# 20242204033/RIS-VEC-MARL

Hardware: AMD Instinct MI355X
Metric: env-steps/sec (all agents) at 8 veh x 64 RIS (higher is better)
Workload: dtype f32

## Files before the change

### ris_vec_marl_amd/csrc/k_step_gen.hip

```cpp
#include <cstddef>

#include "risvec_pipe.hpp"

#ifndef RISVEC_GEN_STORES
#define RISVEC_GEN_STORES kStNonTemporal
#endif

#ifndef RISVEC_GEN_EARLY
#define RISVEC_GEN_EARLY 1
#endif

#ifndef RISVEC_GEN_PRIO
#define RISVEC_GEN_PRIO 1
#endif

#ifndef RISVEC_GEN_STAMPS
#define RISVEC_GEN_STAMPS 0
#endif

namespace risvec {

using GenStores = StorePolicy<RISVEC_GEN_STORES>;
constexpr bool kGenEarlyDraw = RISVEC_GEN_EARLY != 0;
constexpr int kGenPrio = RISVEC_GEN_PRIO;
constexpr bool kGenStamps = RISVEC_GEN_STAMPS != 0;
static_assert(kGenPrio >= 0 && kGenPrio <= 3, "RISVEC_GEN_PRIO: 0 (none) or schedule 1, 2, 3");

constexpr int gen_prio_level(int schedule, int NL, int done) {
    if (schedule == 3) return done < (NL + 1) / 2 ? 1 : 0;
    if (schedule == 2 && done == NL) return 3;
    const int top = NL < 3 ? NL : 3;
    return schedule == 0 || done >= top ? 0 : top - done;
}

constexpr int gen_prio_change(int schedule, int NL, int done) {
    if (schedule == 0) return -1;
    const int now = gen_prio_level(schedule, NL, done);
    return done == 0 || now != gen_prio_level(schedule, NL, done - 1) ? now : -1;
}

template <int V, int M, class Core>
constexpr int gen_prio_of() {
    return std::is_same<Core, MarlCore>::value && V == 8 && M == 64 ? kGenPrio : 0;
}

constexpr int gen_leaf_rank(int G, int NP, int J) {
    auto rev = [](int G_, int j) {
        int r = 0;
        for (int b = 1; b < G_ / 8; b <<= 1) r = (r << 1) | ((j & b) ? 1 : 0);
        return r;
    };
    int rank = 0;
    for (int j = 0; j < G / 8; ++j)
        if (8 * j < NP && rev(G, j) < rev(G, J)) ++rank;
    return rank;
}
constexpr int gen_leaf_count(int G, int NP) { return (NP < G ? NP : G) / 8; }

#if RISVEC_GEN_STAMPS
constexpr int kGenStampSlots = 16, kGenStampMax = 12;
__device__ unsigned long long* g_gen_stamps = nullptr;
__device__ long long g_gen_stamps_waves = 0;
struct GenStamps {
    unsigned long long t[kGenStampMax];
    unsigned long long rt0;
    int n = 0;
    __device__ __forceinline__ void mark() { t[n++] = __builtin_amdgcn_s_memtime(); }
};
#else
struct GenStamps {
    __device__ __forceinline__ void mark() {}
};
#endif

template <int V, int M>
struct GenShape : PipeShape<V, M> {
    using S = PipeShape<V, M>;
    static_assert(M % kGeoChunk == 0, "rows are rebuilt in whole 16-element chunks");
    static_assert(S::EPW * V == kWave, "a group is 64 rows");
    static constexpr int NCH = M / kGeoChunk;
    static_assert(NCH <= kWave, "a pass must cover at least one row");
    static constexpr int RPP = kWave / NCH;
    static constexpr int RPU = S::PC * S::VPP;
    static_assert(RPP % RPU == 0, "a pass must hold whole units");
    static constexpr int UPP = RPP / RPU;
    static constexpr int SP = UPP >= S::CHUNKS ? 1 : S::CHUNKS / UPP;
    static constexpr int EPO = SP * UPP / S::CHUNKS;
    static constexpr int NO = NCH / SP;
    static_assert(SP * UPP % S::CHUNKS == 0 && NCH % SP == 0 && NO * EPO == S::EPW, "outer iterations must tile the group");
    static constexpr int STAGE = kWave * (kGeoChunk / 2 + 1);
};

template <int SP, bool HD>
struct GenRows {
    double ang[SP];
    double2 w[SP];
};
template <int SP>
struct GenRows<SP, true> {
    double2 head[SP];
    double2 w[SP];
};
template <int SP, int EPO, int NIT, bool TK, bool HD>
struct GenFeed : GenRows<SP, HD> {
    float4 t[EPO][NIT];
};
template <int SP, int EPO, int NIT, bool HD>
struct GenFeed<SP, EPO, NIT, true, HD> : GenRows<SP, HD> {
    unsigned k[EPO][NIT];
};

template <class Core>
struct GenArgs {
    Dims d;
    typename Core::Params P;
    typename Core::Args A;
    const double* steer;
    const double* z_r;
    int n_groups_total, per_wave, rev;
};

template <class Core>
__device__ __forceinline__ const GenArgs<Core>& late_args() {
    static_assert(offsetof(GenArgs<Core>, d) == 0 && std::is_trivially_copyable<GenArgs<Core>>::value,
                  "the kernel-argument segment must be the struct itself");
    typedef const __attribute__((address_space(4))) GenArgs<Core>* SegPtr;
    SegPtr seg = (SegPtr)__builtin_amdgcn_kernarg_segment_ptr();
    asm volatile("" : "+s"(seg));
    return *(const GenArgs<Core>*)seg;
}

template <int V, int M, class Core, bool TK, bool ONE, bool HD>
__device__ __forceinline__ void gen_stage_form(const GenArgs<Core>& KA) {
    using In = typename Core::In;
    using S = GenShape<V, M>;
    constexpr int VP = S::VP, EPW = S::EPW, NP = S::NP, G = S::G, NIT = S::NIT, VPP = S::VPP;
    constexpr int PC = S::PC, CHUNKS = S::CHUNKS, K = S::K;
    constexpr int NCH = S::NCH, RPP = S::RPP, RPU = S::RPU, UPP = S::UPP, SP = S::SP, EPO = S::EPO, NO = S::NO;
    static_assert(std::is_same<typename Core::Args, StepArgs>::value, "the GEN members step on StepArgs");
    using Feed = GenFeed<SP, EPO, NIT, TK, HD>;
    __shared__ float s_img[kBlock / kWave][kWave * 2];
    __shared__ float2 s_ph[TK ? kBlock / kWave : 1][16];
    __shared__ float4 s_stage[kBlock / kWave][S::STAGE];

    const Dims& d = KA.d;
    const typename Core::Args& A = KA.A;
    const double* __restrict__ steer = KA.steer;
    const int n_groups_total = KA.n_groups_total;

    const int lane = threadIdx.x & (kWave - 1), wave = threadIdx.x >> 6;
    const int gl = lane % G, gv = lane / G;
    const int wid = __builtin_amdgcn_readfirstlane(blockIdx.x * (kBlock / kWave) + wave);
    const float4* __restrict__ t4 = reinterpret_cast<const float4*>(A.theta);
    const float4* __restrict__ b4 = reinterpret_cast<const float4*>(A.b);
    const double2* __restrict__ z2 = reinterpret_cast<const double2*>(KA.z_r);
    const int e_last = d.E - 1;
    const int row_last = d.E * V - 1;
    float4 bq[NIT];
    int pcl[NIT];
#pragma unroll
    for (int it = 0; it < NIT; ++it) {
        const int p = gl + it * G;
        const float4 x = b4[p < NP ? p : NP - 1];
        bq[it] = p < NP ? x : make_float4(0.f, 0.f, 0.f, 0.f);
        pcl[it] = (NP % G == 0 || p < NP) ? p : NP - 1;
    }
    const int p_row = lane / NCH, p_ch = lane % NCH, p_m0 = p_ch * kGeoChunk;
    float4* __restrict__ stage = s_stage[wave];
    float4* __restrict__ p_dst = stage + lane * (kGeoChunk / 2 + 1);
    const float4* c_src[NIT];
#pragma unroll
    for (int it = 0; it < NIT; ++it) {
        const int f = gv * NP + pcl[it];
        c_src[it] = stage + (f >> 3) * (kGeoChunk / 2 + 1) + (f & 7);
    }

    auto load_feed = [&](Feed& f, int grp, int o) {
#pragma unroll
        for (int sp = 0; sp < SP; ++sp) {
            int row = grp * kWave + (o * SP + sp) * RPP + p_row;
            row = row < row_last ? row : row_last;
            if constexpr (HD) f.head[sp] = reinterpret_cast<const double2*>(steer)[(long long)row * NCH + p_ch];
            else f.ang[sp] = steer[row];
            f.w[sp] = z2[row];
        }
#pragma unroll
        for (int ie = 0; ie < EPO; ++ie) {
            int e = grp * EPW + o * EPO + ie;
            e = e < e_last ? e : e_last;
            if constexpr (TK) {
                const uint8_t* __restrict__ kb = A.theta_k + (long long)e * A.theta_k_stride;
#pragma unroll
                for (int it = 0; it < NIT; ++it) f.k[ie][it] = *reinterpret_cast<const uint16_t*>(kb + 2 * pcl[it]);
            } else {
                const float4* __restrict__ tb = t4 + (long long)e * NP;
#pragma unroll
                for (int it = 0; it < NIT; ++it) f.t[ie][it] = tb[pcl[it]];
            }
        }
    };

    auto do_outer = [&](int o, const Feed& cur) {
        float2 w0[NIT], w1[NIT];
#pragma unroll
        for (int sp = 0; sp < SP; ++sp) {
            float4 q[kGeoChunk / 2];
            if constexpr (HD) steer_chunk_from_head(cur.head[sp].x, cur.head[sp].y, cur.w[sp].x, cur.w[sp].y, q);
            else steer_chunk(cur.ang[sp], cur.w[sp].x, cur.w[sp].y, p_m0, q);
#pragma unroll
            for (int k = 0; k < kGeoChunk / 2; ++k) p_dst[k] = q[k];
            __builtin_amdgcn_wave_barrier();
#pragma unroll
            for (int ul = 0; ul < UPP; ++ul) {
                const int uo = sp * UPP + ul;
                const int c = uo % CHUNKS, ie = uo / CHUNKS;
                if (c == 0) {
#pragma unroll
                    for (int it = 0; it < NIT; ++it) {
                        float2 t0, t1;
                        if constexpr (TK) {
                            t0 = s_ph[wave][cur.k[ie][it] & 15u];
                            t1 = s_ph[wave][(cur.k[ie][it] >> 8) & 15u];
                        } else {
                            t0 = make_float2(cur.t[ie][it].x, cur.t[ie][it].y);
                            t1 = make_float2(cur.t[ie][it].z, cur.t[ie][it].w);
                        }
                        w0[it] = cmul(t0, make_float2(bq[it].x, bq[it].y));
                        w1[it] = cmul(t1, make_float2(bq[it].z, bq[it].w));
                    }
                }
                float val[8];
#pragma unroll
                for (int pc = 0; pc < PC; ++pc) {
                    float2 acc = make_float2(0.f, 0.f);
#pragma unroll
                    for (int it = 0; it < NIT; ++it) {
                        const float4 h = c_src[it][((ul * RPU + pc * VPP) * NCH) * (kGeoChunk / 2 + 1)];
                        acc = cfma(make_float2(h.x, h.y), w0[it], acc);
                        acc = cfma(make_float2(h.z, h.w), w1[it], acc);
                    }
                    val[2 * pc] = acc.x;
                    val[2 * pc + 1] = acc.y;
                }
                treduce<K, G / 2>(val, gl);
                if (gl % S::WSTRIDE == 0) {
                    const int j = gl / S::WSTRIDE;
                    const int v = (c * PC + (j >> 1)) * VPP + gv;
                    const int i = o * EPO + ie;
                    s_img[wave][(i * VP + v) * 2 + (j & 1)] = val[0];
                }
            }
            __builtin_amdgcn_wave_barrier();
        }
    };

    const int v_mine = lane % VP;

    if constexpr (ONE) {
        if constexpr (TK) {
            RISVEC_ARGS_IN_ONE_TRIP("s"(steer), "s"(KA.z_r), "s"(A.theta_k), "s"(A.theta_k_stride), "s"(A.b),
                                    "s"(n_groups_total), "s"(d.E));
        } else {
            RISVEC_ARGS_IN_ONE_TRIP("s"(steer), "s"(KA.z_r), "s"(A.theta), "s"(A.b), "s"(n_groups_total), "s"(d.E));
        }
        const int grp = wid;
        if (grp >= n_groups_total) return;
        Feed cur;
        load_feed(cur, grp, 0);
        if constexpr (TK) {
            theta_table_fill(s_ph[wave], lane);
            __builtin_amdgcn_wave_barrier();
        }
        const int e_mine = grp * EPW + lane / VP;
        const bool active = e_mine < d.E;
        const In in = Core::load(d, A, e_mine, v_mine, active);
        Core::hold(in);
#pragma unroll 1
        for (int o = 0; o + 1 < NO; ++o) {
            Feed nx;
            load_feed(nx, grp, o + 1);
            do_outer(o, cur);
            cur = nx;
        }
        do_outer(NO - 1, cur);

        const GenArgs<Core>& L = late_args<Core>();
        __builtin_amdgcn_wave_barrier();
        const float2 img = *reinterpret_cast<const float2*>(&s_img[wave][lane * 2]);
        Core::template run<VP, GenStores>(L.d, L.P, L.A, e_mine, v_mine, active, img, in);
    } else {
        const int per_wave = KA.per_wave;
        const int nw = gridDim.x * (kBlock / kWave);
        const int stride = per_wave > 0 ? 1 : nw;
        int grp = per_wave > 0 ? wid * per_wave : wid;
        int grp_end = per_wave > 0 ? grp + per_wave : n_groups_total;
        grp_end = grp_end < n_groups_total ? grp_end : n_groups_total;
        if constexpr (TK) {
            RISVEC_ARGS_IN_ONE_TRIP("s"(steer), "s"(KA.z_r), "s"(A.theta_k), "s"(A.theta_k_stride), "s"(A.b),
                                    "s"(n_groups_total), "s"(per_wave), "s"(d.E));
        } else {
            RISVEC_ARGS_IN_ONE_TRIP("s"(steer), "s"(KA.z_r), "s"(A.theta), "s"(A.b), "s"(n_groups_total), "s"(per_wave),
                                    "s"(d.E));
        }
        if (grp >= grp_end) return;
        const int grp_first = grp;
        if (KA.rev) {
            while (grp + stride < grp_end) grp += stride;
        }
        const int step = KA.rev ? -stride : stride;
        Feed cur;
        load_feed(cur, grp, 0);
        if constexpr (TK) {
            theta_table_fill(s_ph[wave], lane);
            __builtin_amdgcn_wave_barrier();
        }

        auto do_group = [&](int g_cur, const In& in, In& in_nx) {
            const int g_nx = g_cur + step;
            const int nxt = (g_nx >= grp_first && g_nx < grp_end) ? g_nx : 0;
            const int e_mine = g_cur * EPW + lane / VP;
            const bool active = e_mine < d.E;
            Core::hold(in);

#pragma unroll 1
            for (int o = 0; o < NO; ++o) {
                Feed nx;
                if (o + 1 < NO) load_feed(nx, g_cur, o + 1);
                else load_feed(nx, nxt, 0);
                do_outer(o, cur);
                cur = nx;
            }
            const GenArgs<Core>& L = late_args<Core>();
            in_nx = Core::load(L.d, L.A, nxt * EPW + lane / VP, v_mine, nxt * EPW + lane / VP < L.d.E);

            __builtin_amdgcn_wave_barrier();
            const float2 img = *reinterpret_cast<const float2*>(&s_img[wave][lane * 2]);
            Core::template run<VP, GenStores>(L.d, L.P, L.A, e_mine, v_mine, active, img, in);
            __builtin_amdgcn_wave_barrier();
        };

        In inA = Core::load(d, A, grp * EPW + lane / VP, v_mine, grp * EPW + lane / VP < d.E), inB;
        while (true) {
            do_group(grp, inA, inB);
            grp += step;
            if (grp < grp_first || grp >= grp_end) break;
            do_group(grp, inB, inA);
            grp += step;
            if (grp < grp_first || grp >= grp_end) break;
        }
    }
}

template <int G, int O, int J, class Leaf>
__device__ __forceinline__ void row_tree_block(float2 (&out)[8], Leaf&& leaf) {
    if constexpr (O == G) {
        leaf(std::integral_constant<int, J>{}, out);
    } else if constexpr (O >= 16) {
        float2 far[8];
        row_tree_block<G, 2 * O, J>(out, leaf);
        row_tree_block<G, 2 * O, J + O / 8>(far, leaf);
#pragma unroll
        for (int k = 0; k < 8; ++k) out[k] = make_float2(out[k].x + far[k].x, out[k].y + far[k].y);
    } else {
        static_assert(O == 8 && J == 0, "below 16 the values of a row sit in one block");
        float2 far[8];
        row_tree_block<G, 16, 0>(out, leaf);
        row_tree_block<G, 16, 1>(far, leaf);
#pragma unroll
        for (int k = 0; k < 8; ++k) out[k] = make_float2(out[k].x + far[7 - k].x, out[k].y + far[7 - k].y);
    }
}

template <int G, class Leaf>
__device__ __forceinline__ float2 row_tree(Leaf&& leaf) {
    static_assert(G == 16 || G == 32 || G == 64, "treduce<K, G/2> starts at distance 8, 16 or 32");
    float2 s[8];
    row_tree_block<G, 8, 0>(s, leaf);
#pragma unroll
    for (int g = 0; g < 4; ++g) s[g] = make_float2(s[g].x + s[7 - g].x, s[g].y + s[7 - g].y);
#pragma unroll
    for (int g = 0; g < 2; ++g) s[g] = make_float2(s[g].x + s[g + 2].x, s[g].y + s[g + 2].y);
    return make_float2(s[0].x + s[1].x, s[0].y + s[1].y);
}

template <int Q>
struct alignas(2 * Q) GenIdx {
    unsigned w[Q / 2];
};

template <int V, int M, class Core, bool TK, bool HD>
__device__ __forceinline__ void gen_row_lane_form(const GenArgs<Core>& KA) {
    using In = typename Core::In;
    using S = GenShape<V, M>;
    constexpr int VP = S::VP, EPW = S::EPW, NP = S::NP, G = S::G, NIT = S::NIT, NCH = S::NCH;
    static_assert(std::is_same<typename Core::Args, StepArgs>::value, "the GEN members step on StepArgs");
    static_assert(VP == V && EPW * V == kWave, "lane = row of the group");
    static_assert(NP % V == 0 && (NP / V) % 2 == 0, "an env's w is made by its V lanes, an even share each");
    static_assert(NP % G == 0 || NIT == 1, "ragged rows: whole blocks past the end of the row");
    constexpr int Q = NP / V;
    constexpr int WS = NP + 1;
    __shared__ float4 s_w[kBlock / kWave][EPW * WS];
    __shared__ float2 s_ph[TK ? kBlock / kWave : 1][16];

    const Dims& d = KA.d;
    const typename Core::Args& A = KA.A;
    const double* __restrict__ steer = KA.steer;
    const int n_groups_total = KA.n_groups_total;

    constexpr int NL = gen_leaf_count(G, NP);
    constexpr int PRIO = gen_prio_of<V, M, Core>();
    [[maybe_unused]] GenStamps ts;
    if constexpr (kGenStamps) {
#if RISVEC_GEN_STAMPS
        ts.rt0 = __builtin_amdgcn_s_memrealtime();
#endif
        ts.mark();
    }

    const int lane = threadIdx.x & (kWave - 1), wave = threadIdx.x >> 6;
    const int wid = __builtin_amdgcn_readfirstlane(blockIdx.x * (kBlock / kWave) + wave);
    constexpr int level0 = gen_prio_change(PRIO, NL, 0);
#define RISVEC_GEN_ENTRY(text, ...)                                                                                        \
    if constexpr (TK) {                                                                                                    \
        asm volatile(text ::"s"(steer), "s"(KA.z_r), "s"(A.theta_k), "s"(A.theta_k_stride), "s"(A.b), "s"(n_groups_total), \
                     "s"(d.E)__VA_ARGS__);                                                                                 \
    } else {                                                                                                               \
        asm volatile(text ::"s"(steer), "s"(KA.z_r), "s"(A.theta), "s"(A.b), "s"(n_groups_total), "s"(d.E)__VA_ARGS__);    \
    }
    if constexpr (level0 >= 0) {
        RISVEC_GEN_ENTRY("s_setprio %[level]", , [level] "n"(level0))
    } else {
        RISVEC_GEN_ENTRY("", )
    }
#undef RISVEC_GEN_ENTRY
    const int grp = wid;
    if (grp >= n_groups_total) return;

    const int v_mine = lane % VP, i_env = lane / VP;
    const int e_mine = grp * EPW + i_env;
    const bool active = e_mine < d.E;
    const int e_ld = active ? e_mine : d.E - 1;
    const int row = e_ld * V + v_mine;
    double2 head[HD ? NCH : 1];
    if constexpr (HD) {
#pragma unroll
        for (int c = 0; c < NCH; ++c) head[c] = reinterpret_cast<const double2*>(steer)[(long long)row * NCH + c];
    } else {
        head[0].x = steer[row];
    }
    const double2 z = reinterpret_cast<const double2*>(KA.z_r)[row];
    GenIdx<Q> kq;
    float4 tq[TK ? 1 : Q], bq[Q];
    if constexpr (TK) {
        kq = *reinterpret_cast<const GenIdx<Q>*>(A.theta_k + (long long)e_ld * A.theta_k_stride + 2 * Q * v_mine);
    } else {
        const float4* __restrict__ tb = reinterpret_cast<const float4*>(A.theta) + (long long)e_ld * NP + Q * v_mine;
#pragma unroll
        for (int i = 0; i < Q; ++i) tq[i] = tb[i];
    }
#pragma unroll
    for (int i = 0; i < Q; ++i) bq[i] = reinterpret_cast<const float4*>(A.b)[Q * v_mine + i];
    if constexpr (TK) {
        theta_table_fill(s_ph[wave], lane);
        __builtin_amdgcn_wave_barrier();
    }
    RISVEC_ARGS_IN_ONE_TRIP("s"(A.action), "s"(A.data_buf), "s"(A.partner), "s"(A.arrivals), "s"(A.n_groups), "s"(A.mec_q),
                            "s"(A.pl), "s"(A.flags), "s"(d.V), "s"(d.env_offset), "s"(A.seed), "s"(A.counter),
                            "s"(KA.P.poisson_cdf[0]), "s"(KA.P.poisson_cdf[1]), "s"(KA.P.poisson_cdf[2]),
                            "s"(KA.P.poisson_cdf[3]), "s"(KA.P.poisson_cdf[4]), "s"(KA.P.poisson_cdf[5]),
                            "s"(KA.P.poisson_cdf[6]), "s"(KA.P.poisson_cdf[7]));
    const In in = Core::load(d, A, e_mine, v_mine, active);
    int arr = 0;
    if constexpr (kGenEarlyDraw) {
        arr = Core::draw(d, KA.P, A, e_mine, v_mine);
        asm volatile("" : "+v"(arr));
    }
    Core::hold(in);
    if constexpr (kGenStamps) {
        if constexpr (TK) asm volatile("" : "+v"(kq.w[0]), "+v"(bq[0].x));
        else asm volatile("" : "+v"(tq[0].x), "+v"(bq[0].x));
        ts.mark();
    }

    float4* __restrict__ wrow = s_w[wave] + i_env * WS;
#pragma unroll
    for (int i = 0; i < Q; ++i) {
        float2 t0, t1;
        if constexpr (TK) {
            const unsigned k2 = kq.w[i / 2] >> (16 * (i & 1));
            t0 = s_ph[wave][k2 & 15u];
            t1 = s_ph[wave][(k2 >> 8) & 15u];
        } else {
            t0 = make_float2(tq[i].x, tq[i].y);
            t1 = make_float2(tq[i].z, tq[i].w);
        }
        const float2 w0 = cmul(t0, make_float2(bq[i].x, bq[i].y));
        const float2 w1 = cmul(t1, make_float2(bq[i].z, bq[i].w));
        wrow[Q * v_mine + i] = make_float4(w0.x, w0.y, w1.x, w1.y);
    }
    __builtin_amdgcn_wave_barrier();

    auto leaf = [&](auto jc, float2 (&acc)[8]) {
        constexpr int J = decltype(jc)::value;
#pragma unroll
        for (int k = 0; k < 8; ++k) acc[k] = make_float2(0.f, 0.f);
        if constexpr (8 * J < NP) {
#pragma unroll
            for (int it = 0; it < NIT; ++it) {
                constexpr int GC = G / 8;
                const int c = J + it * GC;
                float4 q[kGeoChunk / 2];
                if constexpr (HD) steer_chunk_from_head(head[c].x, head[c].y, z.x, z.y, q);
                else steer_chunk(head[0].x, z.x, z.y, c * kGeoChunk, q);
#pragma unroll
                for (int k = 0; k < 8; ++k) {
                    const float4 w = wrow[8 * c + k];
                    acc[k] = cfma(make_float2(q[k].x, q[k].y), make_float2(w.x, w.y), acc[k]);
                    acc[k] = cfma(make_float2(q[k].z, q[k].w), make_float2(w.z, w.w), acc[k]);
                }
#define RISVEC_GEN_FENCE(text, ...)                                                                                            \
    asm volatile(text : "+v"(acc[0].x), "+v"(acc[0].y), "+v"(acc[1].x), "+v"(acc[1].y), "+v"(acc[2].x), "+v"(acc[2].y),       \
                        "+v"(acc[3].x), "+v"(acc[3].y), "+v"(acc[4].x), "+v"(acc[4].y), "+v"(acc[5].x), "+v"(acc[5].y),       \
                        "+v"(acc[6].x), "+v"(acc[6].y), "+v"(acc[7].x), "+v"(acc[7].y)                                        \
                 : __VA_ARGS__                                                                                                \
                 : "memory")
                constexpr int level = gen_prio_change(PRIO, NL, gen_leaf_rank(G, NP, J) + 1);
                if constexpr (level >= 0) {
                    if (it + 1 == NIT) RISVEC_GEN_FENCE("s_setprio %[level]", [level] "n"(level));
                    else RISVEC_GEN_FENCE("", );
                } else {
                    RISVEC_GEN_FENCE("", );
                }
#undef RISVEC_GEN_FENCE
            }
            if constexpr (kGenStamps) ts.mark();
        }
    };
    float2 img = row_tree<G>(leaf);
    if constexpr (kGenStamps) {
        asm volatile("" : "+v"(img.x), "+v"(img.y));
        ts.mark();
    }

    const GenArgs<Core>& L = late_args<Core>();
#if RISVEC_GEN_STAMPS
    {
        int e_late = L.d.E;
        asm volatile("" : "+s"(e_late));
        ts.mark();
    }
#endif
    Core::template run<VP, GenStores, kGenEarlyDraw>(L.d, L.P, L.A, e_mine, v_mine, active, img, in, arr);
#if RISVEC_GEN_STAMPS
    asm volatile("s_waitcnt vmcnt(0)" ::: "memory");
    ts.mark();
    const unsigned long long rt1 = __builtin_amdgcn_s_memrealtime();
    static_assert(NL + 5 <= kGenStampMax, "entry, first wait, NL leaves, tree, late, end");
    unsigned long long* __restrict__ out = g_gen_stamps;
    if (out != nullptr && wid < g_gen_stamps_waves && lane == 0) {
        out += (long long)wid * kGenStampSlots;
#pragma unroll
        for (int i = 0; i < NL + 5; ++i) out[i] = ts.t[i];
        out[12] = ts.rt0;
        out[13] = rt1;
        out[14] = __builtin_amdgcn_s_getreg(20 | (31 << 11));
        out[15] = (unsigned long long)(unsigned)__builtin_amdgcn_s_getreg(4 | (31 << 11))
                  | ((unsigned long long)(NL + 5) << 32);
    }
#endif
}

template <int V, int M>
struct GenRowLane {
    static constexpr bool value = M <= 64;
};

template <int V, int M, class Core, bool TK, bool ONE, bool HD>
__global__ void __launch_bounds__(kBlock)
k_step_fused_gen(GenArgs<Core> KA) {
    if constexpr (ONE && GenRowLane<V, M>::value) gen_row_lane_form<V, M, Core, TK, HD>(KA);
    else gen_stage_form<V, M, Core, TK, ONE, HD>(KA);
}

constexpr int kGenWavesPerCu = 16;

static thread_local int g_gen_per_wave = 0;

template <int V, int M, class Core>
static hipError_t launch_gen(const RisVecState& s, const typename Core::Params& p, const typename Core::Args& a, bool rev,
                             bool heads, hipStream_t st) {
    using S = GenShape<V, M>;
    const int n_groups = (s.n_envs + S::EPW - 1) / S::EPW;
    const int wpb = kBlock / kWave;
    const int forced_waves = forced_forms().pipe_waves;
    long long want_waves = forced_waves > 0 ? forced_waves : (long long)num_cus() * kGenWavesPerCu;
    if (want_waves > n_groups) want_waves = n_groups;
    const long long per_wave = (n_groups + want_waves - 1) / want_waves;
    want_waves = (n_groups + per_wave - 1) / per_wave;
    const unsigned grid = (unsigned)((want_waves + wpb - 1) / wpb);
    const int contiguous = forced_waves > 0 ? (int)per_wave : 0;
    const double* steer = heads ? s.steer_ang + (long long)s.n_envs * s.n_veh : s.steer_ang;
    const GenArgs<Core> ka{dims_of(s), p, a, steer, s.z_r, n_groups, contiguous, rev ? 1 : 0};
    auto go = [&](auto knl) { hipLaunchKernelGGL(knl, dim3(grid), dim3(kBlock), 0, st, ka); };
    const bool one = per_wave == 1;
    auto pick = [&](auto tk, auto hd) {
        if (one) go(k_step_fused_gen<V, M, Core, decltype(tk)::value, true, decltype(hd)::value>);
        else go(k_step_fused_gen<V, M, Core, decltype(tk)::value, false, decltype(hd)::value>);
    };
    if (a.theta_k != nullptr) {
        if (heads) pick(std::true_type{}, std::true_type{});
        else pick(std::true_type{}, std::false_type{});
    } else {
        if (heads) pick(std::false_type{}, std::true_type{});
        else pick(std::false_type{}, std::false_type{});
    }
    g_gen_per_wave = (int)per_wave;
    return hipGetLastError();
}

int last_gen_launch_groups_per_wave() { return g_gen_per_wave; }

#if RISVEC_GEN_STAMPS
extern "C" int risvec_gen_stamps_buffer(void* buf, long long n_waves) {
    unsigned long long* p = static_cast<unsigned long long*>(buf);
    if (buf == nullptr) n_waves = 0;
    hipError_t err = hipDeviceSynchronize();
    if (err == hipSuccess) err = hipMemcpyToSymbol(HIP_SYMBOL(g_gen_stamps_waves), &n_waves, sizeof(n_waves));
    if (err == hipSuccess) err = hipMemcpyToSymbol(HIP_SYMBOL(g_gen_stamps), &p, sizeof(p));
    if (err == hipSuccess) err = hipDeviceSynchronize();
    return (int)err;
}
#endif

template <int V, int M, bool WHOLE = (M % kGeoChunk == 0)>
struct GenMember {
    static hipError_t launch(const RisVecState&, const RisVecParams&, const StepArgs&, bool, bool, bool, hipStream_t) {
        return hipErrorNotSupported;
    }
};
template <int V, int M>
struct GenMember<V, M, true> {
    static hipError_t launch(const RisVecState& s, const RisVecParams& p, const StepArgs& a, bool ring, bool rev, bool heads,
                             hipStream_t st) {
        return ring ? launch_gen<V, M, MarlRingCore<V>>(s, p, a, rev, heads, st)
                    : launch_gen<V, M, MarlCore>(s, p, a, rev, heads, st);
    }
};

hipError_t launch_step_fused_gen(const RisVecState& s, const RisVecParams& p, const StepArgs& a, const StepPlan& pl,
                                 bool rev, bool heads, hipStream_t st) {
    note_pipe_walk(rev ? 1 : 0);
#define RISVEC_X(VV, MM, DD, EMIN, EMAX, T) \
    if (pl.V == VV && pl.M == MM) return GenMember<VV, MM>::launch(s, p, a, pl.ring, rev, heads, st);
    RISVEC_FIXED_SHAPES(RISVEC_X)
#undef RISVEC_X
    return hipErrorNotSupported;
}

__global__ void __launch_bounds__(kBlock)
k_h_r_from_steer(Dims d, const double* __restrict__ steer_ang, const double* __restrict__ z_r, float* __restrict__ out) {
    const int nchunk = d.M / kGeoChunk;
    const long long idx = (long long)blockIdx.x * kBlock + threadIdx.x;
    if (idx >= (long long)d.E * d.V * nchunk) return;
    const long long ev = idx / nchunk;
    const int m0 = (int)(idx % nchunk) * kGeoChunk;
    const double2 w = reinterpret_cast<const double2*>(z_r)[ev];
    float4 q[kGeoChunk / 2];
    steer_chunk(steer_ang[ev], w.x, w.y, m0, q);
    float4* dst = reinterpret_cast<float4*>(out + (ev * d.M + m0) * 2);
#pragma unroll
    for (int k = 0; k < kGeoChunk / 2; ++k) dst[k] = q[k];
}

__global__ void __launch_bounds__(kBlock)
k_steer_heads(Dims d, const double* __restrict__ steer_ang, double2* __restrict__ heads) {
    const int nchunk = d.M / kGeoChunk;
    const long long idx = (long long)blockIdx.x * kBlock + threadIdx.x;
    if (idx >= (long long)d.E * d.V * nchunk) return;
    heads[idx] = steer_head(steer_ang[idx / nchunk], (int)(idx % nchunk) * kGeoChunk);
}

hipError_t launch_steer_heads(const RisVecState& s, double* heads, hipStream_t st) {
    const long long n = (long long)s.n_envs * s.n_veh * (s.n_ris / kGeoChunk);
    hipLaunchKernelGGL(k_steer_heads, dim3((unsigned)((n + kBlock - 1) / kBlock)), dim3(kBlock), 0, st, dims_of(s), s.steer_ang,
                       reinterpret_cast<double2*>(heads));
    return hipGetLastError();
}

hipError_t launch_h_r_from_steer(const RisVecState& s, float* out, hipStream_t st) {
    const long long n = (long long)s.n_envs * s.n_veh * (s.n_ris / kGeoChunk);
    hipLaunchKernelGGL(k_h_r_from_steer, dim3((unsigned)((n + kBlock - 1) / kBlock)), dim3(kBlock), 0, st, dims_of(s),
                       s.steer_ang, s.z_r, out);
    return hipGetLastError();
}

}
```

Measured before the change: 3.099 billion.

## Stagger steer head loads across leaves and defer core input load

Instead of loading all steer heads at kernel entry, each chunk's head is requested a configurable number of leaves ahead of its use inside the row tree. The core input load is moved into the leaf loop at a chosen rank, with its hold placed one leaf later. The aim is to cut peak live registers and spread memory requests so they overlap with the complex FMA work. In exchange, loads may arrive late and stall leaves, and the schedule becomes more intricate. The change is limited to the MARL core at 8 vehicles by 64 RIS with head data.

```diff
diff --git a/ris_vec_marl_amd/csrc/k_step_gen.hip b/ris_vec_marl_amd/csrc/k_step_gen.hip
--- a/ris_vec_marl_amd/csrc/k_step_gen.hip
+++ b/ris_vec_marl_amd/csrc/k_step_gen.hip
@@ -16,6 +16,13 @@
 
 #ifndef RISVEC_GEN_STAMPS
 #define RISVEC_GEN_STAMPS 0
+#endif
+
+#ifndef RISVEC_GEN_HEADS_AHEAD
+#define RISVEC_GEN_HEADS_AHEAD 1
+#endif
+#ifndef RISVEC_GEN_LATE_IN
+#define RISVEC_GEN_LATE_IN 1
 #endif
 
 namespace risvec {
@@ -24,7 +31,10 @@
 constexpr bool kGenEarlyDraw = RISVEC_GEN_EARLY != 0;
 constexpr int kGenPrio = RISVEC_GEN_PRIO;
 constexpr bool kGenStamps = RISVEC_GEN_STAMPS != 0;
+constexpr int kGenHeadsAhead = RISVEC_GEN_HEADS_AHEAD;
+constexpr bool kGenLateIn = RISVEC_GEN_LATE_IN != 0;
 static_assert(kGenPrio >= 0 && kGenPrio <= 3, "RISVEC_GEN_PRIO: 0 (none) or schedule 1, 2, 3");
+static_assert(kGenHeadsAhead >= 0 && kGenHeadsAhead <= 2, "RISVEC_GEN_HEADS_AHEAD: 0 (all at entry), 1 or 2 leaves ahead");
 
 constexpr int gen_prio_level(int schedule, int NL, int done) {
     if (schedule == 3) return done < (NL + 1) / 2 ? 1 : 0;
@@ -56,6 +66,39 @@
     return rank;
 }
 constexpr int gen_leaf_count(int G, int NP) { return (NP < G ? NP : G) / 8; }
+
+constexpr int gen_head_rank(int G, int NP, int D, int c) {
+    const int own = gen_leaf_rank(G, NP, c % (G / 8));
+    return D == 0 || own < D ? -1 : own - D;
+}
+constexpr bool gen_head_schedule_ok(int G, int NP, int D) {
+    const int NL = gen_leaf_count(G, NP);
+    for (int c = 0; c < NP / 8; ++c) {
+        const int own = gen_leaf_rank(G, NP, c % (G / 8));
+        int n = 0;
+        for (int r = -1; r < NL; ++r)
+            if (gen_head_rank(G, NP, D, c) == r) {
+                ++n;
+                if (r >= own) return false;
+                if (D > 0 && (r == -1) != (own < D)) return false;
+            }
+        if (n != 1) return false;
+    }
+    return true;
+}
+
+template <int V, int M, class Core, bool HD>
+constexpr bool gen_ahead_member() {
+    return HD && std::is_same<Core, MarlCore>::value && V == 8 && M == 64;
+}
+template <int V, int M, class Core, bool HD>
+constexpr int gen_heads_ahead_of() {
+    return gen_ahead_member<V, M, Core, HD>() ? kGenHeadsAhead : 0;
+}
+template <int V, int M, class Core, bool HD>
+constexpr bool gen_late_in_of() {
+    return gen_ahead_member<V, M, Core, HD>() && kGenLateIn;
+}
 
 #if RISVEC_GEN_STAMPS
 constexpr int kGenStampSlots = 16, kGenStampMax = 12;
@@ -409,6 +452,11 @@
 
     constexpr int NL = gen_leaf_count(G, NP);
     constexpr int PRIO = gen_prio_of<V, M, Core>();
+    constexpr int D = gen_heads_ahead_of<V, M, Core, HD>();
+    constexpr bool LATE = gen_late_in_of<V, M, Core, HD>();
+    constexpr int IN_RANK = NL < 2 ? NL - 1 : 1;
+    static_assert(gen_head_schedule_ok(G, NP, 0) && gen_head_schedule_ok(G, NP, 1) && gen_head_schedule_ok(G, NP, 2),
+                  "every chunk's head is requested once, below its own leaf's rank");
     [[maybe_unused]] GenStamps ts;
     if constexpr (kGenStamps) {
 #if RISVEC_GEN_STAMPS
@@ -442,12 +490,14 @@
     const int e_ld = active ? e_mine : d.E - 1;
     const int row = e_ld * V + v_mine;
     double2 head[HD ? NCH : 1];
-    if constexpr (HD) {
-#pragma unroll
-        for (int c = 0; c < NCH; ++c) head[c] = reinterpret_cast<const double2*>(steer)[(long long)row * NCH + c];
-    } else {
-        head[0].x = steer[row];
-    }
+    auto request_heads = [&](auto rc) {
+        constexpr int R = decltype(rc)::value;
+#pragma unroll
+        for (int c = 0; c < NCH; ++c)
+            if (gen_head_rank(G, NP, D, c) == R) head[c] = reinterpret_cast<const double2*>(steer)[(long long)row * NCH + c];
+    };
+    if constexpr (HD) request_heads(std::integral_constant<int, -1>{});
+    else head[0].x = steer[row];
     const double2 z = reinterpret_cast<const double2*>(KA.z_r)[row];
     GenIdx<Q> kq;
     float4 tq[TK ? 1 : Q], bq[Q];
@@ -469,13 +519,14 @@
                             "s"(KA.P.poisson_cdf[0]), "s"(KA.P.poisson_cdf[1]), "s"(KA.P.poisson_cdf[2]),
                             "s"(KA.P.poisson_cdf[3]), "s"(KA.P.poisson_cdf[4]), "s"(KA.P.poisson_cdf[5]),
                             "s"(KA.P.poisson_cdf[6]), "s"(KA.P.poisson_cdf[7]));
-    const In in = Core::load(d, A, e_mine, v_mine, active);
+    In in;
+    if constexpr (!LATE) in = Core::load(d, A, e_mine, v_mine, active);
     int arr = 0;
     if constexpr (kGenEarlyDraw) {
         arr = Core::draw(d, KA.P, A, e_mine, v_mine);
         asm volatile("" : "+v"(arr));
     }
-    Core::hold(in);
+    if constexpr (!LATE) Core::hold(in);
     if constexpr (kGenStamps) {
         if constexpr (TK) asm volatile("" : "+v"(kq.w[0]), "+v"(bq[0].x));
         else asm volatile("" : "+v"(tq[0].x), "+v"(bq[0].x));
@@ -502,6 +553,16 @@
 
     auto leaf = [&](auto jc, float2 (&acc)[8]) {
         constexpr int J = decltype(jc)::value;
+        if constexpr (8 * J < NP && ((D > 0 && NL > 1) || LATE)) {
+            constexpr int R = gen_leaf_rank(G, NP, J);
+            if constexpr (LATE && R == IN_RANK) in = Core::load(d, A, e_mine, v_mine, active);
+            if constexpr (D > 0) request_heads(std::integral_constant<int, R>{});
+            if constexpr (HD) {
+                if constexpr (NIT == 1) asm volatile("" ::"v"(head[J].x), "v"(head[J].y) : "memory");
+                else asm volatile("" ::"v"(head[J].x), "v"(head[J].y), "v"(head[J + G / 8].x), "v"(head[J + G / 8].y) : "memory");
+            }
+            if constexpr (LATE && R == IN_RANK + 1) Core::hold(in);
+        }
 #pragma unroll
         for (int k = 0; k < 8; ++k) acc[k] = make_float2(0.f, 0.f);
         if constexpr (8 * J < NP) {
@@ -537,6 +598,7 @@
         }
     };
     float2 img = row_tree<G>(leaf);
+    if constexpr (LATE && IN_RANK + 1 >= NL) Core::hold(in);
     if constexpr (kGenStamps) {
         asm volatile("" : "+v"(img.x), "+v"(img.y));
         ts.mark();
```

Result: faster. 3.238 billion (median of 6 runs) (+4.5%).
